# ylongqi/openrec

Hardware: NVIDIA H100
Metric: bpr_triplets_per_sec (higher is better)
Workload: dtype f32

## Files before the change

### openrec_b200/build.py

```python
from __future__ import annotations

import os
import shutil
import subprocess
import sys

HERE = os.path.dirname(os.path.abspath(__file__))
CSRC = os.path.join(HERE, "csrc")
LIB = os.path.join(CSRC, "liborx.so")
ROOT = os.path.dirname(HERE)

NVCC_FLAGS = [
    "-gencode", "arch=compute_90a,code=sm_90a",
    "-O3", "-lineinfo", "-std=c++17", "--expt-relaxed-constexpr",
    "-Xcompiler", "-fPIC", "-Xcompiler", "-fvisibility=hidden",
]


def _nvcc():
    for cand in (os.environ.get("NVCC"), shutil.which("nvcc"), "/usr/local/cuda/bin/nvcc"):
        if cand and os.path.exists(cand):
            return cand
    raise RuntimeError("nvcc not found (set NVCC=/path/to/nvcc)")


def sources():
    return sorted(os.path.join(CSRC, f) for f in os.listdir(CSRC) if f.endswith(".cu"))


def _stale():
    if not os.path.exists(LIB):
        return True
    t = os.path.getmtime(LIB)
    deps = [os.path.join(CSRC, f) for f in os.listdir(CSRC) if f.endswith((".cu", ".cuh", ".h"))]
    deps.append(os.path.join(ROOT, "include", "orx.h"))
    return any(os.path.getmtime(d) > t for d in deps)


def build(force=False, verbose=False):
    if not force and not _stale():
        return LIB
    nvcc = _nvcc()
    objs = []
    procs = []
    for src in sources():
        obj = src[:-3] + ".o"
        cmd = [nvcc, *NVCC_FLAGS, "-c", src, "-o", obj]
        if verbose:
            cmd.insert(1, "-Xptxas=-v")
        procs.append((src, subprocess.Popen(cmd, stdout=subprocess.PIPE, stderr=subprocess.STDOUT, text=True)))
        objs.append(obj)
    failed = False
    for src, p in procs:
        out, _ = p.communicate()
        if p.returncode != 0:
            failed = True
            sys.stderr.write(f"nvcc failed on {src}:\n{out}\n")
        elif verbose or out.strip():
            sys.stderr.write(out)
    if failed:
        raise RuntimeError("liborx build failed")
    link = [nvcc, "-shared", "-o", LIB, *objs, "-gencode", "arch=compute_90a,code=sm_90a", "-cudart", "static"]
    r = subprocess.run(link, stdout=subprocess.PIPE, stderr=subprocess.STDOUT, text=True)
    if r.returncode != 0:
        raise RuntimeError("liborx link failed:\n" + r.stdout)
    return LIB


if __name__ == "__main__":
    path = build(force="--force" in sys.argv, verbose="--verbose" in sys.argv)
    print(path)
```

### openrec_b200/csrc/orx_common.cuh

```cuda
#pragma once
#include <cuda_runtime.h>
#include <stdint.h>
#include <stdio.h>

#include <functional>
#include <initializer_list>
#include <type_traits>

#include "../../include/orx.h"

void orx_set_error(const char* fmt, ...);

#define ORX_CUDA(call)                                                                         \
  do {                                                                                         \
    cudaError_t e__ = (call);                                                                  \
    if (e__ != cudaSuccess) {                                                                  \
      orx_set_error("%s:%d %s -> %s", __FILE__, __LINE__, #call, cudaGetErrorString(e__));     \
      return ORX_ERR_CUDA;                                                                     \
    }                                                                                          \
  } while (0)

#define ORX_REQUIRE(cond, msg)                                  \
  do {                                                          \
    if (!(cond)) {                                              \
// ... 163 lines not shown
  return ((unsigned long long)epoch << 33) | (unsigned long long)(uint32_t)id;
}

__device__ __forceinline__ uint32_t orx_hash_insert(const OrxHash& t, int32_t id, int mode) {
  const unsigned long long mine = orx_slot_word(t.epoch, id);
  uint32_t h = orx_hash32((uint32_t)id, t.shift);
  while (true) {
    unsigned long long w = __ldcg(t.slots + h);
    if ((uint32_t)(w >> 33) != t.epoch) {
      const unsigned long long old = atomicCAS(t.slots + h, w, mine);
      if (old == w) {
        if (mode == 1) {
          const int d = atomicAdd(t.counter, 1);
          t.didx[h] = d;
          t.did[d] = id;
        }
        return 0u;
      }
      w = old;
    }
    if ((w & ~ORX_DUP_BIT) == mine) {
      if (!(w & ORX_DUP_BIT)) {
        const unsigned long long old = atomicOr(t.slots + h, ORX_DUP_BIT);
        if (mode == 0 && !(old & ORX_DUP_BIT)) {
          const int d = atomicAdd(t.counter, 1);
          t.didx[h] = d;
          t.did[d] = id;
        }
      }
      return 1u;
    }
    h = (h + 1) & t.mask;
  }
}

__device__ __forceinline__ unsigned long long orx_ld_keep(const unsigned long long* p) {
  unsigned long long v;
  asm volatile("{.reg .b64 pol; createpolicy.fractional.L2::evict_last.b64 pol, 1.0;\n"
               " ld.global.nc.L2::cache_hint.u64 %0, [%1], pol;}" : "=l"(v) : "l"(p));
  return v;
}
__device__ __forceinline__ int32_t orx_ld_keep(const int32_t* p) {
  int32_t v;
  asm volatile("{.reg .b64 pol; createpolicy.fractional.L2::evict_last.b64 pol, 1.0;\n"
               " ld.global.nc.L2::cache_hint.b32 %0, [%1], pol;}" : "=r"(v) : "l"(p));
  return v;
}
__device__ __forceinline__ float orx_ld_keep(const float* p) {
  float v;
  asm volatile("{.reg .b64 pol; createpolicy.fractional.L2::evict_last.b64 pol, 1.0;\n"
               " ld.global.cg.L2::cache_hint.f32 %0, [%1], pol;}" : "=f"(v) : "l"(p));
  return v;
}

template <bool DUP_ONLY = false, bool KEEP = false>
__device__ __forceinline__ uint32_t orx_hash_find(const OrxHash& t, int32_t id, int32_t* d) {
  const unsigned long long mine = orx_slot_word(t.epoch, id);
  uint32_t h = orx_hash32((uint32_t)id, t.shift);
  while (true) {
    const unsigned long long w = KEEP ? orx_ld_keep(t.slots + h) : __ldg(t.slots + h);
    if ((w & ~ORX_DUP_BIT) == mine) {
      const bool dup = (w & ORX_DUP_BIT) != 0;
      *d = (!DUP_ONLY || dup) ? (KEEP ? orx_ld_keep(t.didx + h) : __ldg(t.didx + h)) : -1;
      return dup ? 2u : 1u;
    }
    if ((uint32_t)(w >> 33) != t.epoch) {
      *d = -1;
      return 0u;
    }
    h = (h + 1) & t.mask;
  }
}

template <int W>
__device__ __forceinline__ float orx_group_sum(float v) {
#pragma unroll
  for (int o = W / 2; o > 0; o >>= 1) v += __shfl_xor_sync(ORX_FULL, v, o);
  return v;
}

__device__ __forceinline__ float4 orx_ld4(const float* p) { return *reinterpret_cast<const float4*>(p); }
__device__ __forceinline__ void orx_st4(float* p, float4 v) { *reinterpret_cast<float4*>(p) = v; }
__device__ __forceinline__ float4 orx_ld4_stream(const float* p) { return __ldcs(reinterpret_cast<const float4*>(p)); }
__device__ __forceinline__ void orx_st4_stream(float* p, float4 v) { __stcs(reinterpret_cast<float4*>(p), v); }
__device__ __forceinline__ void orx_red4(float* p, float4 v) {
  asm volatile("red.global.add.v4.f32 [%0], {%1, %2, %3, %4};" ::"l"(p), "f"(v.x), "f"(v.y), "f"(v.z), "f"(v.w)
               : "memory");
}

__device__ __forceinline__ void orx_logsig(float y, float* logsig, float* sig_neg) {
  float e = expf(-fabsf(y));
  *logsig = fminf(y, 0.f) - log1pf(e);
  *sig_neg = (y >= 0.f) ? e / (1.f + e) : 1.f / (1.f + e);
}
__device__ __forceinline__ float orx_sigmoid(float y) {
  float e = expf(-fabsf(y));
  return (y >= 0.f) ? 1.f / (1.f + e) : e / (1.f + e);
}


__device__ __forceinline__ float orx_sqrt_fast(float x) {
  float r;
  asm("sqrt.approx.f32 %0, %1;" : "=f"(r) : "f"(x));
  return r;
}
__device__ __forceinline__ float orx_rcp_fast(float x) {
  float r;
  asm("rcp.approx.f32 %0, %1;" : "=f"(r) : "f"(x));
  return r;
}

template <int OPT>
struct OrxOptSlots {
  static constexpr bool S0 = (OPT == ORX_OPT_ADAGRAD || OPT == ORX_OPT_ADAM_LAZY);
  static constexpr bool S1 = (OPT == ORX_OPT_ADAM_LAZY);
  static constexpr bool STAGE_ONLY = (OPT == ORX_OPT_ADAM_DENSE);
};

template <int OPT>
__device__ __forceinline__ float orx_apply(float w, float g, float& s0, float& s1, const OrxOptDev& o) {
  if (OPT == ORX_OPT_SGD) {
    return w - o.lr * g;
  } else if (OPT == ORX_OPT_ADAGRAD) {
    s0 = s0 + g * g;
    return w - o.lr * g * orx_rcp_fast(orx_sqrt_fast(s0) + o.eps);
  } else {
    s0 = o.beta1 * s0 + (1.f - o.beta1) * g;
    s1 = o.beta2 * s1 + (1.f - o.beta2) * g * g;
    return w - o.lr * s0 * orx_rcp_fast(orx_sqrt_fast(s1) + o.eps);
  }
}

template <int OPT>
__device__ __forceinline__ float4 orx_apply4(float4 w, float4 g, float4& s0, float4& s1, const OrxOptDev& o) {
  float4 r;
  r.x = orx_apply<OPT>(w.x, g.x, s0.x, s1.x, o);
  r.y = orx_apply<OPT>(w.y, g.y, s0.y, s1.y, o);
  r.z = orx_apply<OPT>(w.z, g.z, s0.z, s1.z, o);
  r.w = orx_apply<OPT>(w.w, g.w, s0.w, s1.w, o);
  return r;
}

template <int OPT, bool STREAM>
__device__ __forceinline__ void orx_own_or_stage4(bool own, float* W, float* P0, float* P1, int id, float* G, int d,
                                                  int D, int off, float4 w, float4 g, float4& s0, float4& s1,
                                                  const OrxOptDev& o) {
  typedef OrxOptSlots<OPT> SL;
  auto st = [](float* p, float4 v) {
    if (STREAM) orx_st4_stream(p, v);
    else __stcg(reinterpret_cast<float4*>(p), v);
  };
  if (!SL::STAGE_ONLY && own) {
    const int64_t i = (int64_t)id * D + off;
    st(W + i, orx_apply4<OPT>(w, g, s0, s1, o));
    if (SL::S0) st(P0 + i, s0);
    if (SL::S1) st(P1 + i, s1);
  } else {
    orx_red4(G + (int64_t)d * D + off, g);
  }
}

template <int OPT>
__device__ __forceinline__ void orx_update1(float* W, float* P0, float* P1, float w, float g, const OrxOptDev& o) {
  typedef OrxOptSlots<OPT> SL;
  float s0 = SL::S0 ? *P0 : 0.f, s1 = SL::S1 ? *P1 : 0.f;
  *W = orx_apply<OPT>(w, g, s0, s1, o);
// ... 174 lines not shown
```

### openrec_b200/csrc/orx_mlp_tc.cu

```cuda
#include <cuda.h>
#include <stdlib.h>

#include "orx_common.cuh"

namespace {

constexpr int TM = 128, TN = 128, TK = 16;
constexpr int RAW_STAGES = 4, OP_STAGES = 3, GROUP_KB = 4;
constexpr int OP_SBO = (TK / 4) * 128;
constexpr int NCW = 4;
constexpr int THREADS = 3 * 128;
constexpr int RAW_A = TM * TK * 4, RAW_B = TN * TK * 4, RAW_STAGE = RAW_A + RAW_B;
constexpr int OP_A = TM * TK * 4, OP_B = TN * TK * 4, OP_STAGE = 2 * OP_A + 2 * OP_B;
constexpr int SMEM = RAW_STAGES * RAW_STAGE + OP_STAGES * OP_STAGE;
static_assert(TM * (TN + 1) * 4 <= SMEM, "the epilogue tile must fit in the rings");

__device__ __forceinline__ uint32_t smem_u32(const void* p) { return (uint32_t)__cvta_generic_to_shared(p); }

__device__ __forceinline__ uint64_t make_desc(uint32_t saddr) {
  uint64_t d = 0;
  d |= (uint64_t)((saddr & 0x3FFFF) >> 4);
  d |= (uint64_t)(128 >> 4) << 16;
  d |= (uint64_t)(OP_SBO >> 4) << 32;
  return d;
}

#define ORX_D8(i) "+f"(d[i]), "+f"(d[i + 1]), "+f"(d[i + 2]), "+f"(d[i + 3]), "+f"(d[i + 4]), "+f"(d[i + 5]), \
                  "+f"(d[i + 6]), "+f"(d[i + 7])
__device__ __forceinline__ void wgmma_tf32(float (&d)[64], uint64_t adesc, uint64_t bdesc, uint32_t accumulate) {
  asm volatile(
      "{\n\t.reg .pred p;\n\tsetp.ne.b32 p, %66, 0;\n\t"
      "wgmma.mma_async.sync.aligned.m64n128k8.f32.tf32.tf32 "
      "{%0, %1, %2, %3, %4, %5, %6, %7, %8, %9, %10, %11, %12, %13, %14, %15, "
      "%16, %17, %18, %19, %20, %21, %22, %23, %24, %25, %26, %27, %28, %29, %30, %31, "
      "%32, %33, %34, %35, %36, %37, %38, %39, %40, %41, %42, %43, %44, %45, %46, %47, "
      "%48, %49, %50, %51, %52, %53, %54, %55, %56, %57, %58, %59, %60, %61, %62, %63}, "
      "%64, %65, p, 1, 1;\n\t}\n"
      : ORX_D8(0), ORX_D8(8), ORX_D8(16), ORX_D8(24), ORX_D8(32), ORX_D8(40), ORX_D8(48), ORX_D8(56)
      : "l"(adesc), "l"(bdesc), "r"(accumulate)
      : "memory");
}
#undef ORX_D8
__device__ __forceinline__ void fence_operands(float (&d)[64]) {
#pragma unroll
  for (int j = 0; j < 64; ++j) asm volatile("" : "+f"(d[j])::"memory");
}
__device__ __forceinline__ void wgmma_fence() { asm volatile("wgmma.fence.sync.aligned;" ::: "memory"); }
__device__ __forceinline__ void wgmma_commit() { asm volatile("wgmma.commit_group.sync.aligned;" ::: "memory"); }
template <int N>
__device__ __forceinline__ void wgmma_wait() { asm volatile("wgmma.wait_group.sync.aligned %0;" ::"n"(N) : "memory"); }

__device__ __forceinline__ void mbar_init(uint64_t* bar, uint32_t count) {
  asm volatile("mbarrier.init.shared::cta.b64 [%0], %1;" ::"r"(smem_u32(bar)), "r"(count) : "memory");
}
__device__ __forceinline__ void mbar_wait(uint64_t* bar, uint32_t parity) {
  asm volatile(
      "{\n\t.reg .pred p;\n\tWAIT_%=:\n\t"
      "mbarrier.try_wait.parity.shared::cta.b64 p, [%0], %1;\n\t"
      "@p bra DONE_%=;\n\tbra WAIT_%=;\n\tDONE_%=:\n\t}\n" ::"r"(smem_u32(bar)),
      "r"(parity)
      : "memory");
}
__device__ __forceinline__ void mbar_arrive(uint64_t* bar) {
  asm volatile("mbarrier.arrive.shared::cta.b64 _, [%0];" ::"r"(smem_u32(bar)) : "memory");
}
__device__ __forceinline__ void mbar_expect_tx(uint64_t* bar, uint32_t bytes) {
  asm volatile("mbarrier.arrive.expect_tx.shared::cta.b64 _, [%0], %1;" ::"r"(smem_u32(bar)), "r"(bytes) : "memory");
}
__device__ __forceinline__ void tma_load_2d(void* smem_dst, const CUtensorMap* tm, int c0, int c1, uint64_t* bar) {
  asm volatile(
      "cp.async.bulk.tensor.2d.shared::cluster.global.mbarrier::complete_tx::bytes [%0], [%1, {%2, %3}], [%4];" ::"r"(
          smem_u32(smem_dst)),
      "l"(tm), "r"(c0), "r"(c1), "r"(smem_u32(bar))
      : "memory");
}

__device__ __forceinline__ float to_tf32(float v) {
  uint32_t r;
  asm("cvt.rna.tf32.f32 %0, %1;" : "=r"(r) : "f"(v));
  return __uint_as_float(r);
}
__device__ __forceinline__ void split4(const float4 v, float4* hi, float4* lo) {
  hi->x = to_tf32(v.x); lo->x = v.x - hi->x;
  hi->y = to_tf32(v.y); lo->y = v.y - hi->y;
  hi->z = to_tf32(v.z); lo->z = v.z - hi->z;
  hi->w = to_tf32(v.w); lo->w = v.w - hi->w;
}

template <bool KC>
__device__ __forceinline__ void item_offsets(int R, int wi, int lane, int* src_off, int* dst_off) {
  int row, kcore;
  if (KC) {
    row = 8 * wi + (lane & 7);
    kcore = lane >> 3;
    *src_off = row * 64 + ((kcore ^ ((row >> 1) & 3)) << 4);
  } else {
    row = 32 * (wi >> 2) + lane;
    kcore = wi & 3;
    *src_off = (kcore * 4 * R + row) * 4;
  }
  *dst_off = (row >> 3) * OP_SBO + kcore * 128 + (row & 7) * 16;
}
template <bool KC, int R>
__device__ __forceinline__ void convert_item(const unsigned char* raw, int src_off, int dst_off, unsigned char* hi_tile,
                                             unsigned char* lo_tile) {
  float4 v;
  if (KC) {
    v = *reinterpret_cast<const float4*>(raw + src_off);
  } else {
    const float* p = reinterpret_cast<const float*>(raw + src_off);
    v.x = p[0];
    v.y = p[R];
    v.z = p[2 * R];
    v.w = p[3 * R];
  }
  float4 h, l;
  split4(v, &h, &l);
  *reinterpret_cast<float4*>(hi_tile + dst_off) = h;
  *reinterpret_cast<float4*>(lo_tile + dst_off) = l;
}

template <int TA, int TB>
__global__ void __launch_bounds__(THREADS, 1)
k_gemm_tma(const __grid_constant__ CUtensorMap tmA, const __grid_constant__ CUtensorMap tmB, float* __restrict__ C,
           int64_t ldc, int M, int N, int K, const float* __restrict__ bias, int act, float* __restrict__ part) {
  constexpr bool A_KC = TA == 0, B_KC = TB == 1;
  extern __shared__ __align__(1024) unsigned char smem_raw[];
  __shared__ __align__(8) uint64_t raw_full[RAW_STAGES], raw_empty[RAW_STAGES], op_full[OP_STAGES], op_empty[OP_STAGES];
  unsigned char* smem = reinterpret_cast<unsigned char*>((reinterpret_cast<uintptr_t>(smem_raw) + 1023) & ~(uintptr_t)1023);
  const int warp = threadIdx.x >> 5, lane = threadIdx.x & 31;
  const int wgi = __shfl_sync(ORX_FULL, (int)threadIdx.x >> 7, 0);
  const int m0 = blockIdx.y * TM, n0 = blockIdx.x * TN;
  unsigned char* raw_ring = smem;
  unsigned char* op_ring = smem + RAW_STAGES * RAW_STAGE;

  if (threadIdx.x == 0) {
    for (int s = 0; s < RAW_STAGES; ++s) { mbar_init(&raw_full[s], 1); mbar_init(&raw_empty[s], NCW); }
    for (int s = 0; s < OP_STAGES; ++s) { mbar_init(&op_full[s], NCW); mbar_init(&op_empty[s], 8); }
    asm volatile("fence.mbarrier_init.release.cluster;" ::: "memory");
    asm volatile("prefetch.tensormap [%0];" ::"l"(&tmA) : "memory");
    asm volatile("prefetch.tensormap [%0];" ::"l"(&tmB) : "memory");
  }
  __syncthreads();

  const int nkb_all = (K + TK - 1) / TK;
  const int per = (nkb_all + (int)gridDim.z - 1) / (int)gridDim.z;
  const int kb_lo = blockIdx.z * per;
  const int nkb = max(0, min(nkb_all, kb_lo + per) - kb_lo);

  float sum[64];
#pragma unroll
  for (int j = 0; j < 64; ++j) sum[j] = 0.f;

  if (wgi == 0) {
    auto load = [&](int kb) {
      const int rs = kb % RAW_STAGES;
      unsigned char* st = raw_ring + (size_t)rs * RAW_STAGE;
      const int k0 = (kb_lo + kb) * TK;
      mbar_expect_tx(&raw_full[rs], RAW_STAGE);
      if (A_KC) tma_load_2d(st, &tmA, k0, m0, &raw_full[rs]); else tma_load_2d(st, &tmA, m0, k0, &raw_full[rs]);
      if (B_KC) tma_load_2d(st + RAW_A, &tmB, k0, n0, &raw_full[rs]); else tma_load_2d(st + RAW_A, &tmB, n0, k0, &raw_full[rs]);
    };
    const bool producer = warp == 0 && lane == 0;
    if (producer)
      for (int kb = 0; kb < min(nkb, RAW_STAGES - 1); ++kb) load(kb);
    constexpr int ITEMS_A = TM / 8, ITEMS_B = TN / 8;
    constexpr int NIT = (ITEMS_A + ITEMS_B) / NCW;
    static_assert((ITEMS_A + ITEMS_B) % NCW == 0 && ITEMS_A % NCW == 0, "items must divide evenly");
    constexpr int NIT_A = ITEMS_A / NCW;
    int src_off[NIT], dst_off[NIT];
#pragma unroll
    for (int i = 0; i < NIT; ++i) {
      const int wi = warp + NCW * i;
      if (i < NIT_A) item_offsets<A_KC>(TM, wi, lane, &src_off[i], &dst_off[i]);
      else item_offsets<B_KC>(TN, wi - ITEMS_A, lane, &src_off[i], &dst_off[i]);
    }
    for (int kb = 0; kb < nkb; ++kb) {
      const int rs = kb % RAW_STAGES, os = kb % OP_STAGES;
      const int nk = kb + RAW_STAGES - 1;
      if (producer && nk < nkb) {
        if (nk >= RAW_STAGES) mbar_wait(&raw_empty[nk % RAW_STAGES], ((nk / RAW_STAGES) - 1) & 1);
        load(nk);
      }
      __syncwarp();
      mbar_wait(&raw_full[rs], (kb / RAW_STAGES) & 1);
      if (kb >= OP_STAGES) mbar_wait(&op_empty[os], ((kb / OP_STAGES) - 1) & 1);
      const unsigned char* ra = raw_ring + (size_t)rs * RAW_STAGE;
      const unsigned char* rb = ra + RAW_A;
      unsigned char* oa = op_ring + (size_t)os * OP_STAGE;
      unsigned char* ob = oa + 2 * OP_A;
#pragma unroll
      for (int i = 0; i < NIT; ++i) {
        if (i < NIT_A) convert_item<A_KC, TM>(ra, src_off[i], dst_off[i], oa, oa + OP_A);
        else convert_item<B_KC, TN>(rb, src_off[i], dst_off[i], ob, ob + OP_B);
      }
      asm volatile("fence.proxy.async.shared::cta;" ::: "memory");
      __syncwarp();
      if (lane == 0) {
        mbar_arrive(&op_full[os]);
        mbar_arrive(&raw_empty[rs]);
      }
    }
  } else {
    const int wg = wgi - 1;
    float acc[64];
#pragma unroll
    for (int j = 0; j < 64; ++j) acc[j] = 0.f;
    const uint32_t op0 = smem_u32(op_ring);
    auto release = [&](int s) {
      __syncwarp();
      if (lane == 0) mbar_arrive(&op_empty[s]);
    };
    for (int g0 = 0; g0 < nkb; g0 += GROUP_KB) {
      const int g1 = min(nkb, g0 + GROUP_KB);
      for (int kb = g0; kb < g1; ++kb) {
        const int os = kb % OP_STAGES;
        mbar_wait(&op_full[os], (kb / OP_STAGES) & 1);
        const uint32_t a_hi = op0 + (uint32_t)(os * OP_STAGE + wg * 8 * OP_SBO), a_lo = a_hi + OP_A;
        const uint32_t b_hi = op0 + (uint32_t)(os * OP_STAGE + 2 * OP_A), b_lo = b_hi + OP_B;
        wgmma_fence();
#pragma unroll
        for (int ks = 0; ks < TK / 8; ++ks) {
          const uint32_t o = (uint32_t)(ks * 256);
          wgmma_tf32(acc, make_desc(a_hi + o), make_desc(b_hi + o), (kb == g0 && ks == 0) ? 0u : 1u);
          wgmma_tf32(acc, make_desc(a_hi + o), make_desc(b_lo + o), 1u);
          wgmma_tf32(acc, make_desc(a_lo + o), make_desc(b_hi + o), 1u);
        }
        wgmma_commit();
        wgmma_wait<1>();
        if (kb > g0) release((kb - 1) % OP_STAGES);
      }
      wgmma_wait<0>();
      fence_operands(acc);
      release((g1 - 1) % OP_STAGES);
#pragma unroll
      for (int j = 0; j < 64; ++j) sum[j] += acc[j];
    }
  }

  __syncthreads();
  float* tile = reinterpret_cast<float*>(smem);
  if (warp >= NCW) {
    const int r0 = 16 * (warp - NCW) + (lane >> 2), c0 = 2 * (lane & 3);
#pragma unroll
    for (int j = 0; j < 64; ++j) tile[(r0 + 8 * ((j >> 1) & 1)) * (TN + 1) + 8 * (j >> 2) + c0 + (j & 1)] = sum[j];
  }
  __syncthreads();
  const bool split = gridDim.z > 1;
  float* out = split ? part + (size_t)blockIdx.z * (size_t)M * (size_t)N : C;
  const int64_t ldo = split ? (int64_t)N : ldc;
  for (int r = warp; r < TM; r += THREADS / 32) {
    const int m = m0 + r;
    if (m >= M) break;
#pragma unroll
    for (int c = 0; c < TN; c += 32) {
      const int n = n0 + c + lane;
      if (n < N) {
        float x = tile[r * (TN + 1) + c + lane];
        if (!split) {
          x += bias ? bias[n] : 0.f;
          if (act == 1) x = fmaxf(x, 0.f);
          else if (act == 2) x = orx_sigmoid(x);
        }
        out[(int64_t)m * ldo + n] = x;
      }
    }
  }
}

__global__ void __launch_bounds__(256) k_splitk_reduce(const float* __restrict__ part, int S, int M, int N, float* __restrict__ C,
                                                       int64_t ldc, const float* __restrict__ bias, int act) {
  const int64_t i = (int64_t)blockIdx.x * blockDim.x + threadIdx.x;
  if (i >= (int64_t)M * N) return;
  const int m = (int)(i / N), n = (int)(i % N);
  float x = 0.f;
  for (int z = 0; z < S; ++z) x += part[(size_t)z * (size_t)M * (size_t)N + (size_t)i];
  x += bias ? bias[n] : 0.f;
  if (act == 1) x = fmaxf(x, 0.f);
  else if (act == 2) x = orx_sigmoid(x);
  C[(int64_t)m * ldc + n] = x;
}

typedef CUresult (*EncodeTiledFn)(CUtensorMap*, CUtensorMapDataType, cuuint32_t, void*, const cuuint64_t*, const cuuint64_t*,
                                  const cuuint32_t*, const cuuint32_t*, CUtensorMapInterleave, CUtensorMapSwizzle,
                                  CUtensorMapL2promotion, CUtensorMapFloatOOBfill);
EncodeTiledFn encode_fn() {
  static EncodeTiledFn fn = nullptr;
  if (!fn) {
    void* p = nullptr;
    cudaDriverEntryPointQueryResult q;
    if (cudaGetDriverEntryPoint("cuTensorMapEncodeTiled", &p, cudaEnableDefault, &q) == cudaSuccess && q == cudaDriverEntryPointSuccess)
      fn = (EncodeTiledFn)p;
  }
  return fn;
}

int make_map(CUtensorMap* tm, const float* base, int rows, int K, int64_t ld, bool kc, int tile_rows) {
  EncodeTiledFn enc = encode_fn();
  if (!enc) { orx_set_error("cuTensorMapEncodeTiled is not available in this driver"); return ORX_ERR_CUDA; }
  cuuint64_t dims[2], strides[1];
  cuuint32_t box[2], estr[2] = {1, 1};
  if (kc) { dims[0] = (cuuint64_t)K; dims[1] = (cuuint64_t)rows; box[0] = TK; box[1] = (cuuint32_t)tile_rows; }
  else { dims[0] = (cuuint64_t)rows; dims[1] = (cuuint64_t)K; box[0] = (cuuint32_t)tile_rows; box[1] = TK; }
  strides[0] = (cuuint64_t)ld * 4;
  const CUresult r = enc(tm, CU_TENSOR_MAP_DATA_TYPE_FLOAT32, 2, const_cast<float*>(base), dims, strides, box, estr,
                         CU_TENSOR_MAP_INTERLEAVE_NONE, kc ? CU_TENSOR_MAP_SWIZZLE_64B : CU_TENSOR_MAP_SWIZZLE_NONE,
                         CU_TENSOR_MAP_L2_PROMOTION_L2_128B, CU_TENSOR_MAP_FLOAT_OOB_FILL_NONE);
  if (r != CUDA_SUCCESS) { orx_set_error("cuTensorMapEncodeTiled failed (%d)", (int)r); return ORX_ERR_CUDA; }
  return ORX_OK;
}

template <int TA, int TB>
int launch_tma(const CUtensorMap& ta, const CUtensorMap& tb, float* C, int64_t ldc, int M, int N, int K, const float* bias,
               int act, float* part, int S, cudaStream_t st) {
  ORX_CUDA(cudaFuncSetAttribute(k_gemm_tma<TA, TB>, cudaFuncAttributeMaxDynamicSharedMemorySize, SMEM + 1024));
  dim3 grid((N + TN - 1) / TN, (M + TM - 1) / TM, S);
  k_gemm_tma<TA, TB><<<grid, THREADS, SMEM + 1024, st>>>(ta, tb, C, ldc, M, N, K, bias, act, part);
  ORX_LAUNCH_CHECK();
  return ORX_OK;
}

}

int orx_launch_splitk_reduce(const float* part, int S, int M, int N, float* C, int64_t ldc, const float* bias, int act, cudaStream_t st) {
  const int64_t n = (int64_t)M * N;
  k_splitk_reduce<<<(unsigned)((n + 255) / 256), 256, 0, st>>>(part, S, M, N, C, ldc, bias, act);
  ORX_LAUNCH_CHECK();
  return ORX_OK;
}

int orx_launch_gemm_tc(orx_ctx* h, int TA, int TB, const float* A, int64_t lda, const float* Bm, int64_t ldb, float* C,
                       int64_t ldc, int M, int N, int K, const float* bias, int act, cudaStream_t st) {
  if (TA == 1 && TB == 1) return ORX_ERR_UNSUPPORTED;
  if (N < 16 || K < 8 || M < 64) return ORX_ERR_UNSUPPORTED;
  if ((lda & 3) || (ldb & 3) || (((uintptr_t)A | (uintptr_t)Bm) & 15)) return ORX_ERR_UNSUPPORTED;
  const int tiles = ((N + TN - 1) / TN) * ((M + TM - 1) / TM);
  const int nkb = (K + TK - 1) / TK;
  int S = 1;
  const int sms = h->num_sms;
  if (tiles < sms && nkb >= 32) {
    S = (2 * sms + tiles - 1) / tiles;
    if (S > nkb / 8) S = nkb / 8;
    if (S < 1) S = 1;
  }
  int rc;
  float* part = nullptr;
  if (S > 1) {
    if ((rc = orx_grow((void**)&h->splitk, &h->splitk_cap, sizeof(float) * (size_t)S * (size_t)M * (size_t)N))) return rc;
    part = h->splitk;
  }
  CUtensorMap ta, tb;
  if ((rc = make_map(&ta, A, M, K, lda, TA == 0, TM))) return rc;
  if ((rc = make_map(&tb, Bm, N, K, ldb, TB == 1, TN))) return rc;
#define ORX_TMA(a, b) rc = launch_tma<a, b>(ta, tb, C, ldc, M, N, K, bias, act, part, S, st)
  if (TA == 0 && TB == 0) ORX_TMA(0, 0);
  else if (TA == 0) ORX_TMA(0, 1);
  else ORX_TMA(1, 0);
#undef ORX_TMA
  if (rc) return rc;
  orx_log_dispatch(h, ORX_OP_GEMM, ORX_VARIANT_GEMM_TMA, TA, TB, M, N, K, S);
  if (S > 1) return orx_launch_splitk_reduce(part, S, M, N, C, ldc, bias, act, st);
  return ORX_OK;
}
```

### openrec_b200/csrc/orx_pairwise.cu

```cuda
#include "orx_common.cuh"
#include "orx_pair.cuh"

__global__ void k_index_build(OrxHash hu, OrxHash hi, const int32_t* __restrict__ a, int64_t rows_a,
                              const int32_t* __restrict__ b0, const int32_t* __restrict__ b1, int64_t rows_b, int n,
                              int stage_all, int32_t* bad) {
  const int i = blockIdx.x * blockDim.x + threadIdx.x;
  if (i >= (b1 ? 3 : 2) * n) return;
  const int t = i < n ? i : (i < 2 * n ? i - n : i - 2 * n);
  const int32_t ia = a[t], ib0 = b0[t], ib1 = b1 ? b1[t] : 0;
  const bool ga = ia >= 0 && (int64_t)ia < rows_a, gb0 = ib0 >= 0 && (int64_t)ib0 < rows_b,
             gb1 = ib1 >= 0 && (int64_t)ib1 < rows_b;
  const bool all = ga && gb0 && gb1;
  if (i < n) {
    if (!ga) atomicAdd(bad, 1);
    else if (all) orx_hash_insert(hu, ia, stage_all);
  } else {
    const bool g = i < 2 * n ? gb0 : gb1;
    if (!g) atomicAdd(bad, 1);
    else if (all) orx_hash_insert(hi, i < 2 * n ? ib0 : ib1, stage_all);
  }
}

__global__ void k_index_resolve(OrxHash hu, OrxHash hi, const int32_t* __restrict__ uid, const int32_t* __restrict__ pid,
                                const int32_t* __restrict__ nid, int64_t rows_u, int64_t rows_i, int n, int mode,
// ... 12 lines not shown
      const uint32_t cu = orx_hash_find<true>(hu, u, &r.y);
      const uint32_t cp = orx_hash_find<true>(hi, p, &r.z);
      const uint32_t cn = orx_hash_find<true>(hi, q, &r.w);
      r.x = 1 | (cu == 1u ? 2 : 0) | (cp == 1u ? 4 : 0) | (cn == 1u ? 8 : 0);
    }
  }
  res[t] = r;
}

__global__ void k_index_build_strided(OrxHash hu, const int32_t* __restrict__ a, int64_t stride, int64_t rows, int n,
                                       int stage_all, int32_t* bad) {
  for (int i = blockIdx.x * blockDim.x + threadIdx.x; i < n; i += gridDim.x * blockDim.x) {
    const int32_t id = a[(int64_t)i * stride];
    if (id >= 0 && (int64_t)id < rows) orx_hash_insert(hu, id, stage_all);
    else atomicAdd(bad, 1);
  }
}

int orx_launch_index_build_strided(orx_ctx* c, const int32_t* a, int64_t stride, int64_t rows, int32_t n,
                                   bool stage_all, cudaStream_t st) {
  if (n <= 0) return ORX_OK;
  OrxIndexSet& s = c->set[0];
  int rc = orx_take_epoch(s.u, st);
  if (rc) return rc;
  k_index_build_strided<<<(n + 255) / 256, 256, 0, st>>>(s.u, a, stride, rows, n, stage_all ? 1 : 0, s.ctl + 3);
  ORX_LAUNCH_CHECK();
  return ORX_OK;
}

int orx_launch_index_build(orx_ctx* c, const int32_t* a, int64_t rows_a, const int32_t* b0, const int32_t* b1,
                           int64_t rows_b, int32_t n, int mode, cudaStream_t st) {
  const int total = (b1 ? 3 : 2) * n;
  if (total <= 0) return ORX_OK;
  OrxIndexSet& s = c->set[0];
  int rc;
  if ((rc = orx_take_epoch(s.u, st)) || (rc = orx_take_epoch(s.i, st))) return rc;
  k_index_build<<<(total + 255) / 256, 256, 0, st>>>(s.u, s.i, a, rows_a, b0, b1, rows_b, n, mode, s.ctl + 3);
  ORX_LAUNCH_CHECK();
  return ORX_OK;
}

template <int K, bool S0, bool S1>
struct TripRegs {
  float4 u[K], p[K], n[K];
  float4 us0[K], ps0[K], ns0[K];
  float4 us1[K], ps1[K], ns1[K];
  int fl, uu, pp, nn, du, dp, dn;
};

template <int KIND, int OPT, int D, int CH, int MINB, bool PIPE>
__global__ void __launch_bounds__(256, MINB) k_pair_step(const PairArgs a) {
  constexpr int G = (D / 4 < 32) ? D / 4 : 32;
  constexpr int K = D / (4 * G);
  constexpr int TPW = 32 / G;
  typedef OrxOptSlots<OPT> SL;
  static_assert(CH % TPW == 0, "chunk must be a multiple of the triplets per warp");
  typedef TripRegs<K, SL::S0, SL::S1> Regs;

  const int lane = threadIdx.x & 31;
  const int warp = (blockIdx.x * blockDim.x + threadIdx.x) >> 5;
  const int grp = lane / G, gl = lane % G;
  const int t = warp * CH + lane;
  const float4 z4 = make_float4(0.f, 0.f, 0.f, 0.f);
  orx_pdl_wait();

  int u_id = 0, p_id = 0, n_id = 0, du = -1, dp = -1, dn = -1, flags = 0;
  if (lane < CH && t < a.B) {
    u_id = a.uid[t];
    p_id = a.pid[t];
    n_id = a.nid[t];
    if (a.res) {
      const int4 r = __ldcs(a.res + t);
      flags = r.x;
      du = r.y;
      dp = r.z;
      dn = r.w;
    } else {
      flags = (u_id >= 0 && u_id < a.rowsU && p_id >= 0 && p_id < a.rowsI && n_id >= 0 && n_id < a.rowsI) ? 1 : 0;
    }
  }

  auto load_var = [&](int j, Regs& r) {
    const int src = j + grp;
    r.fl = __shfl_sync(ORX_FULL, flags, src) & 1;
    r.uu = __shfl_sync(ORX_FULL, u_id, src);
    r.pp = __shfl_sync(ORX_FULL, p_id, src);
    r.nn = __shfl_sync(ORX_FULL, n_id, src);
#pragma unroll
    for (int k = 0; k < K; ++k) {
      const int off = (k * G + gl) * 4;
      r.u[k] = r.fl ? orx_ld4_stream(a.U + (int64_t)r.uu * D + off) : z4;
      r.p[k] = r.fl ? orx_ld4_stream(a.I + (int64_t)r.pp * D + off) : z4;
      r.n[k] = r.fl ? orx_ld4_stream(a.I + (int64_t)r.nn * D + off) : z4;
    }
  };
  Regs ra, rb;
  load_var(0, ra);
  if (PIPE && TPW < CH) load_var(TPW, rb);

  float bp = 0.f, bn = 0.f, bps0 = 0.f, bps1 = 0.f, bns0 = 0.f, bns1 = 0.f;
  if (flags & 1) {
    uint32_t cu = 0, cp = 0, cn = 0;
    if (!a.res) {
      cu = orx_hash_find<!SL::STAGE_ONLY, true>(a.hu, u_id, &du);
      cp = orx_hash_find<!SL::STAGE_ONLY, true>(a.hi, p_id, &dp);
      cn = orx_hash_find<!SL::STAGE_ONLY, true>(a.hi, n_id, &dn);
    }
    bp = orx_ld_keep(a.Bv + p_id);
    bn = orx_ld_keep(a.Bv + n_id);
    if (!SL::STAGE_ONLY) {
      if (!a.res) flags |= (cu == 1u ? 2 : 0) | (cp == 1u ? 4 : 0) | (cn == 1u ? 8 : 0);
      if (SL::S0) {
        if (flags & 4) bps0 = orx_ld_keep(a.Bs0 + p_id);
        if (flags & 8) bns0 = orx_ld_keep(a.Bs0 + n_id);
      }
      if (SL::S1) {
        if (flags & 4) bps1 = orx_ld_keep(a.Bs1 + p_id);
        if (flags & 8) bns1 = orx_ld_keep(a.Bs1 + n_id);
      }
    }
  }

  auto load_slots = [&](int j, Regs& r) {
    const int src = j + grp;
    r.fl = __shfl_sync(ORX_FULL, flags, src);
    r.du = __shfl_sync(ORX_FULL, du, src);
    r.dp = __shfl_sync(ORX_FULL, dp, src);
    r.dn = __shfl_sync(ORX_FULL, dn, src);
#pragma unroll
    for (int k = 0; k < K; ++k) {
      const int off = (k * G + gl) * 4;
      if (SL::S0) {
        r.us0[k] = (r.fl & 2) ? orx_ld4_stream(a.Us0 + (int64_t)r.uu * D + off) : z4;
        r.ps0[k] = (r.fl & 4) ? orx_ld4_stream(a.Is0 + (int64_t)r.pp * D + off) : z4;
        r.ns0[k] = (r.fl & 8) ? orx_ld4_stream(a.Is0 + (int64_t)r.nn * D + off) : z4;
      }
      if (SL::S1) {
        r.us1[k] = (r.fl & 2) ? orx_ld4_stream(a.Us1 + (int64_t)r.uu * D + off) : z4;
        r.ps1[k] = (r.fl & 4) ? orx_ld4_stream(a.Is1 + (int64_t)r.pp * D + off) : z4;
        r.ns1[k] = (r.fl & 8) ? orx_ld4_stream(a.Is1 + (int64_t)r.nn * D + off) : z4;
      }
    }
  };
  load_slots(0, ra);
  if (PIPE && TPW < CH) load_slots(TPW, rb);

  float loss_acc = 0.f, l2_acc = 0.f, g_own = 0.f;

  auto process = [&](int j, Regs& r) {
    float s1 = 0.f, s2 = 0.f, sq = 0.f;
#pragma unroll
    for (int k = 0; k < K; ++k) {
      if (KIND == ORX_PAIR_BPR) {
        s1 += dot4(r.u[k], r.p[k]);
        s2 += dot4(r.u[k], r.n[k]);
      } else {
        s1 += sqd4(r.u[k], r.p[k]);
        s2 += sqd4(r.u[k], r.n[k]);
      }
      sq += dot4(r.u[k], r.u[k]) + dot4(r.p[k], r.p[k]) + dot4(r.n[k], r.n[k]);
    }
    l2_acc += sq;
    s1 = orx_group_sum<G>(s1);
    s2 = orx_group_sum<G>(s2);
    float lt, g;
    pair_score<KIND>(s1, s2, __shfl_sync(ORX_FULL, bp, j + grp), __shfl_sync(ORX_FULL, bn, j + grp), a.margin, a.c_loss,
                     a.inv_B, &lt, &g);
    const bool v = r.fl & 1;
    if (!v) { lt = 0.f; g = 0.f; }
    if (gl == 0) loss_acc += lt;
    const float gbias = (KIND == ORX_PAIR_BPR) ? g : -g;
#pragma unroll
    for (int q = 0; q < TPW; ++q) {
      const float val = __shfl_sync(ORX_FULL, gbias, q * G);
      if (lane == j + q) g_own = val;
    }
// ... 577 lines not shown
```

Measured before the change: 373.5 million.

## Feed GEMM A operand from registers and choose cache hints for embedding loads

The TF32 GEMM now builds its A-operand hi/lo split inside the consumer warpgroups. Each consumer reads A straight from the raw TMA ring into registers and issues register-sourced wgmma, so the A conversion and its staging buffer are removed. The change also deepens the raw and operand rings, rebalances registers with setmaxnreg, and moves the epilogue tile write. Separately, the BPR kernel now loads embedding rows with an L2-caching load when the resolved flags mark a row as not first-seen, and keeps streaming loads for first-seen rows. A build-script option for out-of-tree builds with defines and GEMM diagnostic macros is added too. The swizzle index math and barrier counts carry correctness risk.

```diff
diff --git a/openrec_b200/build.py b/openrec_b200/build.py
--- a/openrec_b200/build.py
+++ b/openrec_b200/build.py
@@ -37,15 +37,18 @@
     return any(os.path.getmtime(d) > t for d in deps)
 
 
-def build(force=False, verbose=False):
-    if not force and not _stale():
+def build(force=False, verbose=False, out_dir=None, defines=()):
+    if out_dir is None and not force and not _stale():
         return LIB
     nvcc = _nvcc()
+    lib = LIB if out_dir is None else os.path.join(os.path.abspath(out_dir), "liborx.so")
+    if out_dir is not None:
+        os.makedirs(out_dir, exist_ok=True)
     objs = []
     procs = []
     for src in sources():
-        obj = src[:-3] + ".o"
-        cmd = [nvcc, *NVCC_FLAGS, "-c", src, "-o", obj]
+        obj = src[:-3] + ".o" if out_dir is None else os.path.join(os.path.abspath(out_dir), os.path.basename(src)[:-3] + ".o")
+        cmd = [nvcc, *NVCC_FLAGS, *(f"-D{d}" for d in defines), "-c", src, "-o", obj]
         if verbose:
             cmd.insert(1, "-Xptxas=-v")
         procs.append((src, subprocess.Popen(cmd, stdout=subprocess.PIPE, stderr=subprocess.STDOUT, text=True)))
@@ -60,13 +63,19 @@
             sys.stderr.write(out)
     if failed:
         raise RuntimeError("liborx build failed")
-    link = [nvcc, "-shared", "-o", LIB, *objs, "-gencode", "arch=compute_90a,code=sm_90a", "-cudart", "static"]
+    link = [nvcc, "-shared", "-o", lib, *objs, "-gencode", "arch=compute_90a,code=sm_90a", "-cudart", "static"]
     r = subprocess.run(link, stdout=subprocess.PIPE, stderr=subprocess.STDOUT, text=True)
     if r.returncode != 0:
         raise RuntimeError("liborx link failed:\n" + r.stdout)
-    return LIB
+    return lib
 
 
 if __name__ == "__main__":
-    path = build(force="--force" in sys.argv, verbose="--verbose" in sys.argv)
-    print(path)
+    import argparse
+    ap = argparse.ArgumentParser()
+    ap.add_argument("--force", action="store_true")
+    ap.add_argument("--verbose", action="store_true", help="print ptxas register / shared-memory / spill lines")
+    ap.add_argument("--out", default=None, help="build into this directory instead of csrc/")
+    ap.add_argument("-D", dest="defines", action="append", default=[], metavar="NAME=VALUE")
+    a = ap.parse_args()
+    print(build(force=a.force, verbose=a.verbose, out_dir=a.out, defines=a.defines))
diff --git a/openrec_b200/csrc/orx_common.cuh b/openrec_b200/csrc/orx_common.cuh
--- a/openrec_b200/csrc/orx_common.cuh
+++ b/openrec_b200/csrc/orx_common.cuh
@@ -269,6 +269,7 @@
 __device__ __forceinline__ float4 orx_ld4(const float* p) { return *reinterpret_cast<const float4*>(p); }
 __device__ __forceinline__ void orx_st4(float* p, float4 v) { *reinterpret_cast<float4*>(p) = v; }
 __device__ __forceinline__ float4 orx_ld4_stream(const float* p) { return __ldcs(reinterpret_cast<const float4*>(p)); }
+__device__ __forceinline__ float4 orx_ld4_reuse(const float* p) { return __ldcg(reinterpret_cast<const float4*>(p)); }
 __device__ __forceinline__ void orx_st4_stream(float* p, float4 v) { __stcs(reinterpret_cast<float4*>(p), v); }
 __device__ __forceinline__ void orx_red4(float* p, float4 v) {
   asm volatile("red.global.add.v4.f32 [%0], {%1, %2, %3, %4};" ::"l"(p), "f"(v.x), "f"(v.y), "f"(v.z), "f"(v.w)
diff --git a/openrec_b200/csrc/orx_mlp_tc.cu b/openrec_b200/csrc/orx_mlp_tc.cu
--- a/openrec_b200/csrc/orx_mlp_tc.cu
+++ b/openrec_b200/csrc/orx_mlp_tc.cu
@@ -3,16 +3,21 @@
 
 #include "orx_common.cuh"
 
+#ifndef ORX_GEMM_DIAG
+#define ORX_GEMM_DIAG 0
+#endif
+
 namespace {
 
 constexpr int TM = 128, TN = 128, TK = 16;
-constexpr int RAW_STAGES = 4, OP_STAGES = 3, GROUP_KB = 4;
+constexpr int RAW_STAGES = 8, RAW_LEAD = RAW_STAGES - 2, OP_STAGES = 4, GROUP_KB = 4;
 constexpr int OP_SBO = (TK / 4) * 128;
 constexpr int NCW = 4;
 constexpr int THREADS = 3 * 128;
 constexpr int RAW_A = TM * TK * 4, RAW_B = TN * TK * 4, RAW_STAGE = RAW_A + RAW_B;
-constexpr int OP_A = TM * TK * 4, OP_B = TN * TK * 4, OP_STAGE = 2 * OP_A + 2 * OP_B;
+constexpr int OP_B = TN * TK * 4, OP_STAGE = 2 * OP_B;
 constexpr int SMEM = RAW_STAGES * RAW_STAGE + OP_STAGES * OP_STAGE;
+constexpr int A_BOX_T = 32;
 static_assert(TM * (TN + 1) * 4 <= SMEM, "the epilogue tile must fit in the rings");
 
 __device__ __forceinline__ uint32_t smem_u32(const void* p) { return (uint32_t)__cvta_generic_to_shared(p); }
@@ -27,17 +32,17 @@
 
 #define ORX_D8(i) "+f"(d[i]), "+f"(d[i + 1]), "+f"(d[i + 2]), "+f"(d[i + 3]), "+f"(d[i + 4]), "+f"(d[i + 5]), \
                   "+f"(d[i + 6]), "+f"(d[i + 7])
-__device__ __forceinline__ void wgmma_tf32(float (&d)[64], uint64_t adesc, uint64_t bdesc, uint32_t accumulate) {
+__device__ __forceinline__ void wgmma_tf32_rs(float (&d)[64], const uint32_t (&a)[4], uint64_t bdesc, uint32_t accumulate) {
   asm volatile(
-      "{\n\t.reg .pred p;\n\tsetp.ne.b32 p, %66, 0;\n\t"
+      "{\n\t.reg .pred p;\n\tsetp.ne.b32 p, %69, 0;\n\t"
       "wgmma.mma_async.sync.aligned.m64n128k8.f32.tf32.tf32 "
       "{%0, %1, %2, %3, %4, %5, %6, %7, %8, %9, %10, %11, %12, %13, %14, %15, "
       "%16, %17, %18, %19, %20, %21, %22, %23, %24, %25, %26, %27, %28, %29, %30, %31, "
       "%32, %33, %34, %35, %36, %37, %38, %39, %40, %41, %42, %43, %44, %45, %46, %47, "
       "%48, %49, %50, %51, %52, %53, %54, %55, %56, %57, %58, %59, %60, %61, %62, %63}, "
-      "%64, %65, p, 1, 1;\n\t}\n"
+      "{%64, %65, %66, %67}, %68, p, 1, 1;\n\t}\n"
       : ORX_D8(0), ORX_D8(8), ORX_D8(16), ORX_D8(24), ORX_D8(32), ORX_D8(40), ORX_D8(48), ORX_D8(56)
-      : "l"(adesc), "l"(bdesc), "r"(accumulate)
+      : "r"(a[0]), "r"(a[1]), "r"(a[2]), "r"(a[3]), "l"(bdesc), "r"(accumulate)
       : "memory");
 }
 #undef ORX_D8
@@ -45,11 +50,26 @@
 #pragma unroll
   for (int j = 0; j < 64; ++j) asm volatile("" : "+f"(d[j])::"memory");
 }
+template <int N>
+__device__ __forceinline__ void fence_operands(uint32_t (&a)[N]) {
+#pragma unroll
+  for (int j = 0; j < N; ++j) asm volatile("" : "+r"(a[j])::"memory");
+}
+template <int R>
+__device__ __forceinline__ void setmaxnreg_dec() { asm volatile("setmaxnreg.dec.sync.aligned.u32 %0;" ::"n"(R)); }
+template <int R>
+__device__ __forceinline__ void setmaxnreg_inc() { asm volatile("setmaxnreg.inc.sync.aligned.u32 %0;" ::"n"(R)); }
+__device__ __forceinline__ void bar_sync_all(int id) { asm volatile("bar.sync %0, %1;" ::"r"(id), "n"(THREADS) : "memory"); }
 __device__ __forceinline__ void wgmma_fence() { asm volatile("wgmma.fence.sync.aligned;" ::: "memory"); }
 __device__ __forceinline__ void wgmma_commit() { asm volatile("wgmma.commit_group.sync.aligned;" ::: "memory"); }
 template <int N>
 __device__ __forceinline__ void wgmma_wait() { asm volatile("wgmma.wait_group.sync.aligned %0;" ::"n"(N) : "memory"); }
 
+__device__ __forceinline__ float lds_f32(uint32_t saddr) {
+  float v;
+  asm volatile("ld.shared.f32 %0, [%1];" : "=f"(v) : "r"(saddr) : "memory");
+  return v;
+}
 __device__ __forceinline__ void mbar_init(uint64_t* bar, uint32_t count) {
   asm volatile("mbarrier.init.shared::cta.b64 [%0], %1;" ::"r"(smem_u32(bar)), "r"(count) : "memory");
 }
@@ -118,6 +138,12 @@
   split4(v, &h, &l);
   *reinterpret_cast<float4*>(hi_tile + dst_off) = h;
   *reinterpret_cast<float4*>(lo_tile + dst_off) = l;
+}
+
+template <int TA>
+__device__ __forceinline__ int tile_row(int f) {
+  if (TA == 0) return f;
+  return (f & 3) | (((f >> 2) & 1) << 4) | (((f >> 3) & 1) << 2) | (((f >> 4) & 1) << 3) | (f & 0x60);
 }
 
 template <int TA, int TB>
@@ -135,7 +161,7 @@
   unsigned char* op_ring = smem + RAW_STAGES * RAW_STAGE;
 
   if (threadIdx.x == 0) {
-    for (int s = 0; s < RAW_STAGES; ++s) { mbar_init(&raw_full[s], 1); mbar_init(&raw_empty[s], NCW); }
+    for (int s = 0; s < RAW_STAGES; ++s) { mbar_init(&raw_full[s], 1); mbar_init(&raw_empty[s], NCW + 8); }
     for (int s = 0; s < OP_STAGES; ++s) { mbar_init(&op_full[s], NCW); mbar_init(&op_empty[s], 8); }
     asm volatile("fence.mbarrier_init.release.cluster;" ::: "memory");
     asm volatile("prefetch.tensormap [%0];" ::"l"(&tmA) : "memory");
@@ -148,36 +174,33 @@
   const int kb_lo = blockIdx.z * per;
   const int nkb = max(0, min(nkb_all, kb_lo + per) - kb_lo);
 
-  float sum[64];
-#pragma unroll
-  for (int j = 0; j < 64; ++j) sum[j] = 0.f;
-
   if (wgi == 0) {
+    setmaxnreg_dec<56>();
     auto load = [&](int kb) {
       const int rs = kb % RAW_STAGES;
       unsigned char* st = raw_ring + (size_t)rs * RAW_STAGE;
       const int k0 = (kb_lo + kb) * TK;
       mbar_expect_tx(&raw_full[rs], RAW_STAGE);
-      if (A_KC) tma_load_2d(st, &tmA, k0, m0, &raw_full[rs]); else tma_load_2d(st, &tmA, m0, k0, &raw_full[rs]);
+      if (A_KC) {
+        tma_load_2d(st, &tmA, k0, m0, &raw_full[rs]);
+      } else {
+#pragma unroll
+        for (int q = 0; q < TM / A_BOX_T; ++q) tma_load_2d(st + q * (A_BOX_T * TK * 4), &tmA, m0 + q * A_BOX_T, k0, &raw_full[rs]);
+      }
       if (B_KC) tma_load_2d(st + RAW_A, &tmB, k0, n0, &raw_full[rs]); else tma_load_2d(st + RAW_A, &tmB, n0, k0, &raw_full[rs]);
     };
     const bool producer = warp == 0 && lane == 0;
     if (producer)
-      for (int kb = 0; kb < min(nkb, RAW_STAGES - 1); ++kb) load(kb);
-    constexpr int ITEMS_A = TM / 8, ITEMS_B = TN / 8;
-    constexpr int NIT = (ITEMS_A + ITEMS_B) / NCW;
-    static_assert((ITEMS_A + ITEMS_B) % NCW == 0 && ITEMS_A % NCW == 0, "items must divide evenly");
-    constexpr int NIT_A = ITEMS_A / NCW;
+      for (int kb = 0; kb < min(nkb, RAW_LEAD); ++kb) load(kb);
+    constexpr int ITEMS_B = TN / 8;
+    constexpr int NIT = ITEMS_B / NCW;
+    static_assert(ITEMS_B % NCW == 0, "items must divide evenly");
     int src_off[NIT], dst_off[NIT];
 #pragma unroll
-    for (int i = 0; i < NIT; ++i) {
-      const int wi = warp + NCW * i;
-      if (i < NIT_A) item_offsets<A_KC>(TM, wi, lane, &src_off[i], &dst_off[i]);
-      else item_offsets<B_KC>(TN, wi - ITEMS_A, lane, &src_off[i], &dst_off[i]);
-    }
+    for (int i = 0; i < NIT; ++i) item_offsets<B_KC>(TN, warp + NCW * i, lane, &src_off[i], &dst_off[i]);
     for (int kb = 0; kb < nkb; ++kb) {
       const int rs = kb % RAW_STAGES, os = kb % OP_STAGES;
-      const int nk = kb + RAW_STAGES - 1;
+      const int nk = kb + RAW_LEAD;
       if (producer && nk < nkb) {
         if (nk >= RAW_STAGES) mbar_wait(&raw_empty[nk % RAW_STAGES], ((nk / RAW_STAGES) - 1) & 1);
         load(nk);
@@ -185,15 +208,12 @@
       __syncwarp();
       mbar_wait(&raw_full[rs], (kb / RAW_STAGES) & 1);
       if (kb >= OP_STAGES) mbar_wait(&op_empty[os], ((kb / OP_STAGES) - 1) & 1);
-      const unsigned char* ra = raw_ring + (size_t)rs * RAW_STAGE;
-      const unsigned char* rb = ra + RAW_A;
-      unsigned char* oa = op_ring + (size_t)os * OP_STAGE;
-      unsigned char* ob = oa + 2 * OP_A;
-#pragma unroll
-      for (int i = 0; i < NIT; ++i) {
-        if (i < NIT_A) convert_item<A_KC, TM>(ra, src_off[i], dst_off[i], oa, oa + OP_A);
-        else convert_item<B_KC, TN>(rb, src_off[i], dst_off[i], ob, ob + OP_B);
-      }
+      const unsigned char* rb = raw_ring + (size_t)rs * RAW_STAGE + RAW_A;
+      unsigned char* ob = op_ring + (size_t)os * OP_STAGE;
+#if ORX_GEMM_DIAG != 2
+#pragma unroll
+      for (int i = 0; i < NIT; ++i) convert_item<B_KC, TN>(rb, src_off[i], dst_off[i], ob, ob + OP_B);
+#endif
       asm volatile("fence.proxy.async.shared::cta;" ::: "memory");
       __syncwarp();
       if (lane == 0) {
@@ -201,11 +221,29 @@
         mbar_arrive(&raw_empty[rs]);
       }
     }
+    bar_sync_all(1);
   } else {
+    setmaxnreg_inc<224>();
     const int wg = wgi - 1;
-    float acc[64];
-#pragma unroll
-    for (int j = 0; j < 64; ++j) acc[j] = 0.f;
+    const int f0 = 64 * wg + 16 * (warp & 3) + (lane >> 2), t = lane & 3;
+    int aoff[4];
+#pragma unroll
+    for (int i = 0; i < 4; ++i) {
+      if (A_KC) {
+        const int r = f0, c = i;
+        aoff[i] = r * 64 + ((c ^ ((r >> 1) & 3)) << 4) + t * 4;
+      } else {
+        const int h = i >> 1, e = i & 1, m = tile_row<TA>(f0 + 8 * e), k = t + 4 * h;
+        aoff[i] = (m / A_BOX_T) * (A_BOX_T * TK * 4) + k * (A_BOX_T * 4) + ((((m % A_BOX_T) >> 2) ^ (k & 7)) << 4) + (m & 3) * 4;
+      }
+    }
+    auto a_off = [&](int ks, int h, int e) {
+      return A_KC ? aoff[2 * ks + h] + 512 * e : aoff[2 * h + e] + 1024 * ks;
+    };
+    float acc[64], sum[64];
+#pragma unroll
+    for (int j = 0; j < 64; ++j) acc[j] = sum[j] = 0.f;
+    uint32_t fa[2][TK / 8][2][4];
     const uint32_t op0 = smem_u32(op_ring);
     auto release = [&](int s) {
       __syncwarp();
@@ -213,39 +251,63 @@
     };
     for (int g0 = 0; g0 < nkb; g0 += GROUP_KB) {
       const int g1 = min(nkb, g0 + GROUP_KB);
-      for (int kb = g0; kb < g1; ++kb) {
-        const int os = kb % OP_STAGES;
+#pragma unroll
+      for (int j = 0; j < GROUP_KB; ++j) {
+        const int kb = g0 + j;
+        if (kb >= g1) break;
+        const int rs = kb % RAW_STAGES, os = kb % OP_STAGES;
+        auto& f = fa[j & 1];
+        mbar_wait(&raw_full[rs], (kb / RAW_STAGES) & 1);
+        const uint32_t ra = smem_u32(raw_ring) + (uint32_t)(rs * RAW_STAGE);
+#pragma unroll
+        for (int ks = 0; ks < TK / 8; ++ks)
+#pragma unroll
+          for (int q = 0; q < 4; ++q) {
+            const float v = lds_f32(ra + (uint32_t)a_off(ks, q >> 1, q & 1));
+            const float hi = to_tf32(v);
+            f[ks][0][q] = __float_as_uint(hi);
+            f[ks][1][q] = __float_as_uint(v - hi);
+          }
+        __syncwarp();
+        if (lane == 0) mbar_arrive(&raw_empty[rs]);
         mbar_wait(&op_full[os], (kb / OP_STAGES) & 1);
-        const uint32_t a_hi = op0 + (uint32_t)(os * OP_STAGE + wg * 8 * OP_SBO), a_lo = a_hi + OP_A;
-        const uint32_t b_hi = op0 + (uint32_t)(os * OP_STAGE + 2 * OP_A), b_lo = b_hi + OP_B;
+        const uint32_t b_hi = op0 + (uint32_t)(os * OP_STAGE), b_lo = b_hi + OP_B;
         wgmma_fence();
+#if ORX_GEMM_DIAG != 1
 #pragma unroll
         for (int ks = 0; ks < TK / 8; ++ks) {
           const uint32_t o = (uint32_t)(ks * 256);
-          wgmma_tf32(acc, make_desc(a_hi + o), make_desc(b_hi + o), (kb == g0 && ks == 0) ? 0u : 1u);
-          wgmma_tf32(acc, make_desc(a_hi + o), make_desc(b_lo + o), 1u);
-          wgmma_tf32(acc, make_desc(a_lo + o), make_desc(b_hi + o), 1u);
+          wgmma_tf32_rs(acc, f[ks][0], make_desc(b_hi + o), (j == 0 && ks == 0) ? 0u : 1u);
+          wgmma_tf32_rs(acc, f[ks][0], make_desc(b_lo + o), 1u);
+          wgmma_tf32_rs(acc, f[ks][1], make_desc(b_hi + o), 1u);
         }
+#endif
         wgmma_commit();
         wgmma_wait<1>();
-        if (kb > g0) release((kb - 1) % OP_STAGES);
+        if (j > 0) {
+#pragma unroll
+          for (int ks = 0; ks < TK / 8; ++ks) { fence_operands(fa[(j - 1) & 1][ks][0]); fence_operands(fa[(j - 1) & 1][ks][1]); }
+          release((kb - 1) % OP_STAGES);
+        }
       }
       wgmma_wait<0>();
       fence_operands(acc);
+#pragma unroll
+      for (int b = 0; b < 2; ++b)
+#pragma unroll
+        for (int ks = 0; ks < TK / 8; ++ks) { fence_operands(fa[b][ks][0]); fence_operands(fa[b][ks][1]); }
       release((g1 - 1) % OP_STAGES);
 #pragma unroll
       for (int j = 0; j < 64; ++j) sum[j] += acc[j];
     }
-  }
-
+    bar_sync_all(1);
+    float* tile = reinterpret_cast<float*>(smem);
+    const int c0 = 2 * (lane & 3);
+#pragma unroll
+    for (int j = 0; j < 64; ++j) tile[tile_row<TA>(f0 + 8 * ((j >> 1) & 1)) * (TN + 1) + 8 * (j >> 2) + c0 + (j & 1)] = sum[j];
+  }
   __syncthreads();
-  float* tile = reinterpret_cast<float*>(smem);
-  if (warp >= NCW) {
-    const int r0 = 16 * (warp - NCW) + (lane >> 2), c0 = 2 * (lane & 3);
-#pragma unroll
-    for (int j = 0; j < 64; ++j) tile[(r0 + 8 * ((j >> 1) & 1)) * (TN + 1) + 8 * (j >> 2) + c0 + (j & 1)] = sum[j];
-  }
-  __syncthreads();
+  const float* tile = reinterpret_cast<const float*>(smem);
   const bool split = gridDim.z > 1;
   float* out = split ? part + (size_t)blockIdx.z * (size_t)M * (size_t)N : C;
   const int64_t ldo = split ? (int64_t)N : ldc;
@@ -295,16 +357,18 @@
   return fn;
 }
 
-int make_map(CUtensorMap* tm, const float* base, int rows, int K, int64_t ld, bool kc, int tile_rows) {
+int make_map(CUtensorMap* tm, const float* base, int rows, int K, int64_t ld, bool kc, int box_rows) {
   EncodeTiledFn enc = encode_fn();
   if (!enc) { orx_set_error("cuTensorMapEncodeTiled is not available in this driver"); return ORX_ERR_CUDA; }
   cuuint64_t dims[2], strides[1];
   cuuint32_t box[2], estr[2] = {1, 1};
-  if (kc) { dims[0] = (cuuint64_t)K; dims[1] = (cuuint64_t)rows; box[0] = TK; box[1] = (cuuint32_t)tile_rows; }
-  else { dims[0] = (cuuint64_t)rows; dims[1] = (cuuint64_t)K; box[0] = (cuuint32_t)tile_rows; box[1] = TK; }
+  if (kc) { dims[0] = (cuuint64_t)K; dims[1] = (cuuint64_t)rows; box[0] = TK; box[1] = (cuuint32_t)box_rows; }
+  else { dims[0] = (cuuint64_t)rows; dims[1] = (cuuint64_t)K; box[0] = (cuuint32_t)box_rows; box[1] = TK; }
+  const CUtensorMapSwizzle swz = kc ? CU_TENSOR_MAP_SWIZZLE_64B
+                                    : box_rows * 4 == 128 ? CU_TENSOR_MAP_SWIZZLE_128B : CU_TENSOR_MAP_SWIZZLE_NONE;
   strides[0] = (cuuint64_t)ld * 4;
   const CUresult r = enc(tm, CU_TENSOR_MAP_DATA_TYPE_FLOAT32, 2, const_cast<float*>(base), dims, strides, box, estr,
-                         CU_TENSOR_MAP_INTERLEAVE_NONE, kc ? CU_TENSOR_MAP_SWIZZLE_64B : CU_TENSOR_MAP_SWIZZLE_NONE,
+                         CU_TENSOR_MAP_INTERLEAVE_NONE, swz,
                          CU_TENSOR_MAP_L2_PROMOTION_L2_128B, CU_TENSOR_MAP_FLOAT_OOB_FILL_NONE);
   if (r != CUDA_SUCCESS) { orx_set_error("cuTensorMapEncodeTiled failed (%d)", (int)r); return ORX_ERR_CUDA; }
   return ORX_OK;
@@ -350,7 +414,7 @@
     part = h->splitk;
   }
   CUtensorMap ta, tb;
-  if ((rc = make_map(&ta, A, M, K, lda, TA == 0, TM))) return rc;
+  if ((rc = make_map(&ta, A, M, K, lda, TA == 0, TA == 0 ? TM : A_BOX_T))) return rc;
   if ((rc = make_map(&tb, Bm, N, K, ldb, TB == 1, TN))) return rc;
 #define ORX_TMA(a, b) rc = launch_tma<a, b>(ta, tb, C, ldc, M, N, K, bias, act, part, S, st)
   if (TA == 0 && TB == 0) ORX_TMA(0, 0);
diff --git a/openrec_b200/csrc/orx_pairwise.cu b/openrec_b200/csrc/orx_pairwise.cu
--- a/openrec_b200/csrc/orx_pairwise.cu
+++ b/openrec_b200/csrc/orx_pairwise.cu
@@ -118,16 +118,20 @@
 
   auto load_var = [&](int j, Regs& r) {
     const int src = j + grp;
-    r.fl = __shfl_sync(ORX_FULL, flags, src) & 1;
+    const int f = __shfl_sync(ORX_FULL, flags, src);
+    r.fl = f & 1;
     r.uu = __shfl_sync(ORX_FULL, u_id, src);
     r.pp = __shfl_sync(ORX_FULL, p_id, src);
     r.nn = __shfl_sync(ORX_FULL, n_id, src);
+    const bool ku = a.res && !(f & 2), kp = a.res && !(f & 4), kn = a.res && !(f & 8);
 #pragma unroll
     for (int k = 0; k < K; ++k) {
       const int off = (k * G + gl) * 4;
-      r.u[k] = r.fl ? orx_ld4_stream(a.U + (int64_t)r.uu * D + off) : z4;
-      r.p[k] = r.fl ? orx_ld4_stream(a.I + (int64_t)r.pp * D + off) : z4;
-      r.n[k] = r.fl ? orx_ld4_stream(a.I + (int64_t)r.nn * D + off) : z4;
+      const float *pu = a.U + (int64_t)r.uu * D + off, *pp = a.I + (int64_t)r.pp * D + off,
+                  *pn = a.I + (int64_t)r.nn * D + off;
+      r.u[k] = r.fl ? (ku ? orx_ld4_reuse(pu) : orx_ld4_stream(pu)) : z4;
+      r.p[k] = r.fl ? (kp ? orx_ld4_reuse(pp) : orx_ld4_stream(pp)) : z4;
+      r.n[k] = r.fl ? (kn ? orx_ld4_reuse(pn) : orx_ld4_stream(pn)) : z4;
     }
   };
   Regs ra, rb;
```

New measurement: 375.2 million, median of 6. No clear change (+0.5%).
